# marqo-ai/marqo

Measured on AMD Instinct MI355X. Metric: embeddings/sec, higher is better.
Workload: dtype bf16; 1 GPU; open_clip ViT-B/32 image tower, uint8 224x224 resident in HBM (tower-only), batch 256/GPU; global_batch=256, parallelism=dp1 (replicated weights, sharded items, RCCL all_gather of embeddings), weights=random-init (seed 0) ViT-B-32, last_block_rows=pooled

## Files before the change

include/marqo_hip.h:

```cpp
#ifndef MARQO_HIP_H
#define MARQO_HIP_H

#include <stddef.h>
#include <stdint.h>

#ifdef __cplusplus
extern "C" {
#endif

#define MQ_OK 0
#define MQ_ERR_INVALID (-1)
#define MQ_ERR_HIP (-2)
#define MQ_ERR_WORKSPACE (-3)
#define MQ_ERR_UNSUPPORTED (-4)

#define MQ_ABI_VERSION 15

#define MQ_ACT_NONE 0
#define MQ_ACT_GELU 1
#define MQ_ACT_QUICKGELU 2
#define MQ_ACT_SILU 3
#define MQ_ACT_RELU 4

#define MQ_MASK_NONE 0
// ... 254 lines not shown
int mq_attention_stats(const void* d_qkv, void* d_out, const int32_t* d_cu_seqlens, int64_t nseq, int32_t fixed_len, int32_t max_len, int32_t W,
                       int32_t heads, int32_t mask, float* d_row_part, int64_t rows, void* stream);
int mq_attention_proj_ok(int64_t nseq, int32_t fixed_len, int32_t W, int32_t heads);
int mq_attention_proj(const void* d_qkv, const void* d_w, const float* d_bias, void* d_x, float* d_rowstats, int64_t nseq, int32_t fixed_len, int32_t W,
                      int32_t heads, float eps, const void* d_pf_a, size_t pf_a_bytes, const void* d_pf_b, size_t pf_b_bytes, void* stream);
int mq_panel_gemm_ln_ok(int64_t nseq, int32_t fixed_len, int64_t N, int64_t K);
int mq_panel_gemm_ln(const void* d_x, const void* d_W, const float* d_bias, const float* d_colsum, const float* d_rowstats, void* d_out, int64_t ldc,
                     int64_t nseq, int32_t fixed_len, int64_t N, int64_t K, int flags, void* stream);
int64_t mq_gemm_band_counters(int64_t M);
int mq_gemm_bf16_rsf(const void* d_A, int64_t lda, const void* d_W, int64_t ldw, const float* d_bias, const void* d_residual, void* d_out, int64_t ldc,
                     int64_t M, int64_t N, int64_t K, int flags, float* d_partials, float* d_stats, float eps, uint32_t* d_band_ctr,
                     const void* d_pf_a, size_t pf_a_bytes, const void* d_pf_b, size_t pf_b_bytes, void* stream);
int mq_row_stats(const void* d_x_bf16, float* d_stats, int64_t rows, int32_t W, float eps, void* stream);
int mq_gemm_bf16_ln(const void* d_A, int64_t lda, const void* d_W, int64_t ldw, const float* d_bias, const float* d_colsum, const float* d_rowstats,
                    void* d_out, int64_t ldc, int64_t M, int64_t N, int64_t K, int flags, void* stream);

int mq_layernorm(const float* d_x, const int32_t* d_row_idx, const float* d_g, const float* d_b,
                 void* d_out_bf16, float* d_out_f32, int64_t rows, int32_t W, float eps, void* stream);
int mq_layernorm_ex(const void* d_x, int x_bf16, const int32_t* d_row_idx, const float* d_g, const float* d_b,
                    void* d_out_bf16, float* d_out_f32, int64_t rows, int32_t W, float eps, void* stream);

int mq_attention(const void* d_qkv, void* d_out, const int32_t* d_cu_seqlens, int64_t nseq,
                 int32_t fixed_len, int32_t max_len, int32_t W, int32_t heads, int32_t mask,
                 void* stream);

int mq_attention_bias(const void* d_qkv, void* d_out, const int32_t* d_cu_seqlens, int64_t nseq, int32_t fixed_len,
                      int32_t max_len, int32_t W, int32_t heads, const float* d_rel_bias, int32_t rel_span, void* stream);

int mq_attention_ex(const void* d_qkv, void* d_out, const int32_t* d_cu_seqlens, int64_t nseq,
                    int32_t fixed_len, int32_t max_len, int32_t W, int32_t heads, int32_t mask,
// ... 497 lines not shown
```

marqo_amd/_lib.py:

```python
from __future__ import annotations

import ctypes as C
import os
import re
import subprocess
import sys
import sysconfig
import threading
from typing import Optional
from pathlib import Path

PKG_DIR = Path(__file__).resolve().parent
CSRC_DIR = PKG_DIR / "csrc"
LIB_DIR = PKG_DIR / "lib"
LIB_PATH = Path(os.environ["MARQO_AMD_LIB"]) if os.environ.get("MARQO_AMD_LIB") else LIB_DIR / "libmarqo_hip.so"
HEADER_PATH = PKG_DIR.parent / "include" / "marqo_hip.h"
TORCH_OPS_SRC = CSRC_DIR / "torch_ops.cpp"
TORCH_OPS_PATH = LIB_DIR / "libmarqo_torch_ops.so"
STAGE_SRC = CSRC_DIR / "py_stage.cpp"
STAGE_PATH = LIB_DIR / "_mq_stage.so"

MQ_OK = 0
NO_SCRATCH_UNITS = ("rowops", "gemm_bf16", "gemm_wd", "gemm_fp8", "gemm_small", "attention", "attention_window", "attention_gqa", "attention_gqa256", "attention_relbias", "attn_proj", "panel_gemm", "embed", "convnext", "resnet", "patch_attn", "rerank", "owl_head", "temporal", "audio", "video")
ABI_VERSION = 15
# ... 222 lines not shown
    "mq_vit_workspace_bytes": (C.c_size_t, [C.POINTER(VitCfg), C.c_int64]),
    "mq_clip_text_workspace_bytes": (C.c_size_t, [C.POINTER(ClipTextCfg), C.c_int64, C.c_int64]),
    "mq_bert_workspace_bytes": (C.c_size_t, [C.POINTER(BertCfg), C.c_int64, C.c_int64]),
    "mq_encode_image_u8": (C.c_int, [C.POINTER(VitCfg), C.POINTER(VitWeights), _P, C.c_int64, _P, C.c_int, _P, C.c_size_t, _P]),
    "mq_encode_image_f32": (C.c_int, [C.POINTER(VitCfg), C.POINTER(VitWeights), _P, C.c_int64, _P, C.c_int, _P, C.c_size_t, _P]),
    "mq_encode_clip_text": (C.c_int, [C.POINTER(ClipTextCfg), C.POINTER(ClipTextWeights), _P, _P, _P, C.c_int64, _P, _P,
                                      C.c_int, _P, C.c_size_t, _P]),
    "mq_encode_bert": (C.c_int, [C.POINTER(BertCfg), C.POINTER(BertWeights), _P, _P, _P, C.c_int64, _P, C.c_int, _P,
                                 C.c_size_t, _P]),
    "mq_gemm_bf16": (C.c_int, [_P, C.c_int64, _P, C.c_int64, _P, _P, _P, C.c_int64, C.c_int64, C.c_int64, C.c_int64,
                               C.c_int, _P]),
    "mq_gemm_small_bf16": (C.c_int, [_P, C.c_int64, _P, C.c_int64, _P, _P, _P, C.c_int64, C.c_int64, C.c_int64, C.c_int64, C.c_int, _P]),
    "mq_ln_gemm_small_bf16": (C.c_int, [_P, C.c_int64, C.c_int, _P, _P, C.c_float, _P, C.c_int64, _P, _P, C.c_int64, C.c_int64, C.c_int64,
                                        C.c_int64, C.c_int, _P, _P]),
    "mq_gemm_bf16_ln": (C.c_int, [_P, C.c_int64, _P, C.c_int64, _P, _P, _P, _P, C.c_int64, C.c_int64, C.c_int64, C.c_int64, C.c_int, _P]),
    "mq_row_stats": (C.c_int, [_P, _P, C.c_int64, C.c_int32, C.c_float, _P]),
    "mq_row_stats_finalize": (C.c_int, [_P, C.c_int32, _P, C.c_int64, C.c_int32, C.c_float, _P]),
    "mq_gemm_bf16_lnrs": (C.c_int, [_P, C.c_int64, _P, C.c_int64, _P, _P, _P, _P, _P, C.c_int64, C.c_int64, C.c_int64, C.c_int64, C.c_int, _P, _P]),
    "mq_attention_stats": (C.c_int, [_P, _P, _P, C.c_int64, C.c_int32, C.c_int32, C.c_int32, C.c_int32, C.c_int32, _P, C.c_int64, _P]),
    "mq_attention_proj_ok": (C.c_int, [C.c_int64, C.c_int32, C.c_int32, C.c_int32]),
    "mq_panel_gemm_ln_ok": (C.c_int, [C.c_int64, C.c_int32, C.c_int64, C.c_int64]),
    "mq_panel_gemm_ln": (C.c_int, [_P, _P, _P, _P, _P, _P, C.c_int64, C.c_int64, C.c_int32, C.c_int64, C.c_int64, C.c_int, _P]),
    "mq_attention_proj": (C.c_int, [_P, _P, _P, _P, _P, C.c_int64, C.c_int32, C.c_int32, C.c_int32, C.c_float, _P, C.c_size_t, _P, C.c_size_t, _P]),
    "mq_gemm_bf16_rs": (C.c_int, [_P, C.c_int64, _P, C.c_int64, _P, _P, _P, C.c_int64, C.c_int64, C.c_int64, C.c_int64, C.c_int, _P, _P]),
    "mq_check_device": (C.c_int, [C.c_int]),
    "mq_gemm_band_counters": (C.c_int64, [C.c_int64]),
    "mq_gemm_bf16_rsf": (C.c_int, [_P, C.c_int64, _P, C.c_int64, _P, _P, _P, C.c_int64, C.c_int64, C.c_int64, C.c_int64, C.c_int, _P, _P, C.c_float, _P,
                                   _P, C.c_size_t, _P, C.c_size_t, _P]),
    "mq_gemm_fp8": (C.c_int, [_P, C.c_int64, _P, C.c_int64, _P, C.c_int, _P, _P, _P, _P, C.c_int64, _P, _P, C.c_int64, C.c_int64,
                              C.c_int64, C.c_int, _P]),
# ... 387 lines not shown
```

marqo_amd/csrc/attention.hip:

```cpp
#include <type_traits>
#include "attention_core.h"
#include "knobs.h"

namespace {

#ifndef MQ_ATTN_WAVES_PER_EU
#define MQ_ATTN_WAVES_PER_EU 5
#endif
#if MQ_ATTN_WAVES_PER_EU > 0
#define MQ_ATTN_OCC __attribute__((amdgpu_waves_per_eu(HD == 64 ? MQ_ATTN_WAVES_PER_EU : 1, 8)))
#else
#define MQ_ATTN_OCC
#endif
template <int MASK, bool OUT_FP8, int HD, int HS, int NW, bool BIAS = false>
__global__ __launch_bounds__(NW * 64) MQ_ATTN_OCC void attention_kernel(
    const bf16_t* __restrict__ qkv, void* __restrict__ out_v, const int32_t* __restrict__ cu,
    int fixed_len, int W, int heads, int kpad, float scale_log2e, const float* __restrict__ out_scale, float* amax_out,
    const float* __restrict__ rel_bias = nullptr, int rel_span = 0, int band = 0, float2* __restrict__ row_part = nullptr, int64_t part_ld = 0) {
    bf16_t* out = (bf16_t*)out_v;
    extern __shared__ __attribute__((aligned(16))) char smem[];
    static_assert(HS <= HD && HS % 16 == 0 && (HD == 64 || HD == 128), "head stride: multiple of 16, at most the LDS row");
    constexpr int RB = HD * 2;
    constexpr int NC = HD / 8;
    constexpr int NCS = HS / 8;
    constexpr int NKK = (HS + 31) / 32;
    constexpr int NDT = HS / 16;
    char* sK = smem;
    char* sV = smem + (size_t)kpad * RB;

// ... 6 lines not shown
    const int ld = 3 * W;
    const bf16_t* qb = qkv + (int64_t)row0 * ld + h * HS;
    const bf16_t* kb = qb + W;
    const bf16_t* vb = qb + 2 * W;
    const int nkt = (len + 63) >> 6;
    const int kp = nkt << 6;
    const int lane = threadIdx.x & 63, wave = __builtin_amdgcn_readfirstlane(threadIdx.x >> 6);

    const int nchunks = (kp + kpad - 1) / kpad;
    auto stage = [&](int c) {
        const int base = c * kpad;
        attn_stage_piece<RB, NC, NC - 1, NW, NCS>(sK, sV, kb, vb, ld, base, kp - base < kpad ? kp - base : kpad, len, lane, wave);
    };
    if (nchunks == 1) stage(0);
    const int l15 = lane & 15, g = lane >> 4;
    const int nqb = (len + 15) >> 4;
    float amax_local = 0.f;
    auto load_q = [&](int qr, int kk) -> bf16x8 {
        const int col = 8 * g + 32 * kk;
        if (HS % 32 != 0 && col >= HS) return bf16x8{0, 0, 0, 0, 0, 0, 0, 0};
        return *(const bf16x8*)(qb + (int64_t)qr * ld + col);
    };
    bf16x8 qn[NKK];
    {
        const int q0 = wave * 16 + l15;
        const int qr = q0 < len ? q0 : len - 1;
#pragma unroll
        for (int kk = 0; kk < NKK; ++kk) qn[kk] = load_q(qr, kk);
    }
    asm volatile("s_waitcnt vmcnt(0)" ::: "memory");
    __syncthreads();

    const int vkey = 4 * g + (l15 >> 2);
    const int vcol = (l15 & 3) >> 1, vhalf = (l15 & 1) << 3;

    const int nrounds = (nqb + NW - 1) / NW;
    for (int rnd = 0; rnd < nrounds; ++rnd) {
        const int qblk = rnd * NW + wave;
        const bool active = qblk < nqb;
        if (nchunks == 1 && !active) break;
        const int q = qblk * 16 + l15;
// ... 36 lines not shown
#pragma unroll
                for (int t = 0; t < 4; ++t)
#pragma unroll
                    for (int r = 0; r < 4; ++r) {
                        const int key = kt * 64 + t * 16 + g * 4 + r;
                        sc[t][r] += rb[key < len ? key : len - 1];
                    }
            }
            attn_mask_causal<MASK>(sc, kt, nkt, g, q, qblk * 16, len);
            attn_softmax_step<NDT>(sc, m_run, l_run, o, scale_log2e);
            attn_pv_tile<RB, NDT, NC - 1>(sV, kt, cb, vkey, vcol, vhalf, sc, o);
        }
        }
        if (!active) continue;
        const float inv = attn_inv_denominator(l_run);
        if (q < len) {
            if (OUT_FP8) {
                const float qs = 1.0f / out_scale[0];
                uint8_t* orow8 = (uint8_t*)out_v + (int64_t)(row0 + q) * W + h * HS + 4 * g;
#pragma unroll
                for (int dt = 0; dt < NDT; ++dt) {
                    float v[4];
#pragma unroll
                    for (int e = 0; e < 4; ++e) {
                        v[e] = o[dt][e] * inv;
                        amax_local = fmaxf(amax_local, fabsf(v[e]));
                        v[e] = fminf(fmaxf(v[e] * qs, -448.f), 448.f);
                    }
                    int w = __builtin_amdgcn_cvt_pk_fp8_f32(v[0], v[1], 0, false);
                    w = __builtin_amdgcn_cvt_pk_fp8_f32(v[2], v[3], w, true);
                    *(int*)(orow8 + dt * 16) = w;
// ... 29 lines not shown
        }
    }
    if (OUT_FP8 && amax_out) {
        amax_local = wave_max(amax_local);
        if (lane == 0) atomicMax((int*)amax_out, __float_as_int(amax_local));
    }
}


}


static int attention_impl(const void* d_qkv, void* d_out, const int32_t* d_cu_seqlens, int64_t nseq,
                          int32_t fixed_len, int32_t max_len, int32_t W, int32_t heads, int32_t mask,
                          int32_t out_fp8, const float* d_out_scale, float* d_amax, const float* d_rel_bias, int32_t rel_span, void* stream,
                          float* d_row_part = nullptr, int64_t part_ld = 0) {
    ATTN_ARG_PTRS("mq_attention", d_qkv, d_out);
    MQ_CHECK_ARG(!d_row_part || (!out_fp8 && !d_rel_bias), "mq_attention_stats: bf16 output, no relative-position bias");
    MQ_CHECK_ARG(heads >= 1 && W % heads == 0, "mq_attention: W=%d is not a multiple of heads=%d", W, heads);
    const int hs = W / heads;
    MQ_CHECK_ARG(hs == 64 || hs == 96 || hs == 112 || hs == 128, "mq_attention: head dim must be 64, 96, 112 or 128 (W=%d heads=%d)", W, heads);
    const int hd = hs == 64 ? 64 : 128;
    ATTN_ARG_SEQS("mq_attention", fixed_len, d_cu_seqlens);
    MQ_CHECK_ARG(mask == MQ_MASK_NONE || mask == MQ_MASK_CAUSAL || mask == MQ_MASK_CAUSAL_CLS, "mq_attention: bad mask %d", mask);
    MQ_CHECK_ARG(mask != MQ_MASK_CAUSAL_CLS || !out_fp8, "mq_attention: MQ_MASK_CAUSAL_CLS runs with bf16 output only");
    if (nseq <= 0) return MQ_OK;
    const int maxl = fixed_len > 0 ? fixed_len : max_len;
    ATTN_ARG_MAXL("mq_attention", maxl);
    MQ_CHECK_ARG(!d_rel_bias || (hs == 64 && mask == MQ_MASK_NONE && !out_fp8 && rel_span >= maxl),
                 "mq_attention_bias: the relative-position bias runs with 64-wide heads, no mask, bf16 output and rel_span (%d) >= the longest "
                 "sequence (%d)", rel_span, maxl);
    ATTN_ARG_GRID("mq_attention", nseq * heads);
    const int kpad = attn_kpad(maxl, hd == 64 ? 640 : 320);
    const size_t lds = (size_t)kpad * hd * 4;
    hipStream_t s = (hipStream_t)stream;
    const bool five = mq_attention_waves == 5 && maxl > 64 && maxl <= 80 && hs == 64 && !d_rel_bias;
    const int knob_waves = mq_attention_waves;
    const int nw = five ? 5 : (knob_waves == 4 || knob_waves == 8 ? knob_waves : (maxl > 128 ? 8 : 4));
    const float scale_log2e = 1.44269504088896340736f / sqrtf((float)hs);
    MqProfScope prof(2, s);
    auto launch = [&](auto kern) -> int {
        if (lds > 64 * 1024) {
            hipError_t e = hipFuncSetAttribute((const void*)kern, hipFuncAttributeMaxDynamicSharedMemorySize, (int)lds);
            if (e != hipSuccess) { mq_set_error("mq_attention: hipFuncSetAttribute: %s", hipGetErrorString(e)); return MQ_ERR_HIP; }
        }
        hipLaunchKernelGGL(kern, dim3((unsigned)(nseq * heads)), dim3(nw * 64), lds, s, (const bf16_t*)d_qkv,
                           d_out, d_cu_seqlens, (int)fixed_len, (int)W, (int)heads, kpad, scale_log2e, d_out_scale, d_amax, d_rel_bias, (int)rel_span,
                           (mq_xcd_band && nseq * heads >= 2048) ? 1 : 0, (float2*)d_row_part, part_ld);
        return MQ_OK;
    };
    if (d_rel_bias) {
        const int rcb = nw == 8 ? launch(attention_kernel<MQ_MASK_NONE, false, 64, 64, 8, true>) : launch(attention_kernel<MQ_MASK_NONE, false, 64, 64, 4, true>);
        if (rcb != MQ_OK) return rcb;
        MQ_CHECK_LAUNCH("mq_attention_bias");
        return MQ_OK;
    }
    MQ_CHECK_ARG(!out_fp8 || d_out_scale, "mq_attention: fp8 output needs an out_scale");
    int rc;
    auto pick_nw = [&](auto hd_tag, auto hs_tag, auto nw_tag) -> int {
        constexpr int HD_ = decltype(hd_tag)::value, HS_ = decltype(hs_tag)::value, NW_ = decltype(nw_tag)::value;
        if (out_fp8) return (mask == MQ_MASK_CAUSAL) ? launch(attention_kernel<MQ_MASK_CAUSAL, true, HD_, HS_, NW_>) : launch(attention_kernel<MQ_MASK_NONE, true, HD_, HS_, NW_>);
        if (mask == MQ_MASK_CAUSAL_CLS) return launch(attention_kernel<MQ_MASK_CAUSAL_CLS, false, HD_, HS_, NW_>);
        return (mask == MQ_MASK_CAUSAL) ? launch(attention_kernel<MQ_MASK_CAUSAL, false, HD_, HS_, NW_>) : launch(attention_kernel<MQ_MASK_NONE, false, HD_, HS_, NW_>);
    };
    auto pick = [&](auto hd_tag, auto hs_tag) -> int {
        if constexpr (decltype(hd_tag)::value == 64)
            if (nw == 5) return pick_nw(hd_tag, hs_tag, std::integral_constant<int, 5>{});
        return nw == 8 ? pick_nw(hd_tag, hs_tag, std::integral_constant<int, 8>{}) : pick_nw(hd_tag, hs_tag, std::integral_constant<int, 4>{});
    };
    using std::integral_constant;
    switch (hs) {
        case 64: rc = pick(integral_constant<int, 64>{}, integral_constant<int, 64>{}); break;
        case 96: rc = pick(integral_constant<int, 128>{}, integral_constant<int, 96>{}); break;
// ... 15 lines not shown
                                 int32_t max_len, int32_t W, int32_t heads, const float* d_rel_bias, int32_t rel_span, void* stream) {
    MQ_CHECK_ARG(d_rel_bias, "mq_attention_bias: null bias table");
    return attention_impl(d_qkv, d_out, d_cu_seqlens, nseq, fixed_len, max_len, W, heads, MQ_MASK_NONE, 0, nullptr, nullptr, d_rel_bias, rel_span, stream);
}

extern "C" int mq_attention(const void* d_qkv, void* d_out, const int32_t* d_cu_seqlens, int64_t nseq, int32_t fixed_len,
                            int32_t max_len, int32_t W, int32_t heads, int32_t mask, void* stream) {
    return mq_attention_ex(d_qkv, d_out, d_cu_seqlens, nseq, fixed_len, max_len, W, heads, mask, 0, nullptr, nullptr, stream);
}

extern "C" int mq_attention_stats(const void* d_qkv, void* d_out, const int32_t* d_cu_seqlens, int64_t nseq, int32_t fixed_len, int32_t max_len, int32_t W,
                                  int32_t heads, int32_t mask, float* d_row_part, int64_t rows, void* stream) {
    MQ_CHECK_ARG(d_row_part && rows >= 1 && (fixed_len <= 0 || rows == nseq * fixed_len), "mq_attention_stats: null partials / rows does not match the sequences");
    return attention_impl(d_qkv, d_out, d_cu_seqlens, nseq, fixed_len, max_len, W, heads, mask, 0, nullptr, nullptr, nullptr, 0, stream, d_row_part, rows);
}
```

marqo_amd/csrc/gemm_bf16.hip:

```cpp
#include <map>
#include <mutex>
#include <type_traits>
#include "common.h"
#include "gemm_epilogue.h"
#include "gemm_loop.h"
#include "gemm_sched.h"

bool mq_gemm_small_ok(int64_t M, int64_t N, int64_t K, bool ln);
bool mq_gemm_small_grouped_ok(int64_t M, int64_t N, int64_t K);
int mq_gemm_small(const void* d_A, int64_t lda, const void* d_W, int64_t ldw, const float* d_bias, const void* d_residual, void* d_out,
                  int64_t ldc, int64_t M, int64_t N, int64_t K, int flags, hipStream_t s);
int mq_gemm_wd_launch(int flags, int mt, int ns, const void* A, int64_t lda, const void* W, int64_t ldw, const float* bias, const float* residual, void* out,
                      int64_t ldc, int M, int N, int K, const GemmGeom& g, int wide, const GemmLn& ln, hipStream_t s);

int mq_device_ok();

namespace {

struct GemmSk {
    float* partials;
    unsigned* flags;
    unsigned epoch;
    int tail_splits;
};
// ... 332 lines not shown
        w.partials = (float*)p;
        w.flags = (unsigned*)((char*)p + (size_t)RESIDENT_SLOTS_WIDE * SK_SLOT_BYTES);
        if (hipError_t e = hipMemsetAsync(w.flags, 0, 4096, s); e != hipSuccess) {
            mq_set_error("mq_gemm_bf16: tail workspace memset: %s", hipGetErrorString(e));
            return MQ_ERR_HIP;
        }
    }
    if (++w.epoch == 0) w.epoch = 1;
    out.partials = w.partials;
    out.flags = w.flags;
    out.epoch = w.epoch;
    return MQ_OK;
}

GemmLn ln_rows_from(GemmLn ln, int64_t r, int64_t bands) {
    if (ln.rowstats) ln.rowstats += r;
    if (ln.partials) ln.partials += r;
    if (ln.band_ctr) { ln.band_ctr += bands; ln.stats_out += r; }
    return ln;
}

template <int FLAGS, int MT, int NH = 1, int ORD = 2, int WM = 2>
int launch_gemm_mt(const void* A, int64_t lda, const void* W, int64_t ldw, const float* bias, const float* residual, void* out, int64_t ldc,
                   int M, int N, int K, hipStream_t s, const GemmLn& ln) {
    constexpr int BM = 16 * MT * WM, BN = 128 * NH;
    constexpr int LDS = 2 * (BM + BN) * BK * 2;
    constexpr int SLOTS = (NH == 1 && WM == 2) ? RESIDENT_SLOTS : RESIDENT_SLOTS_WIDE;
    static std::atomic<uint64_t> attr_done{0};
    auto kern = gemm_nt_kernel<FLAGS, MT, NH, WM, ORD>;
    if (hipError_t e = mq_ensure_dyn_lds((const void*)kern, LDS, attr_done); e != hipSuccess) {
        mq_set_error("mq_gemm_bf16: hipFuncSetAttribute: %s", hipGetErrorString(e));
// ... 150 lines not shown
        MQ_GEMM_CASE(MQ_EPI_BIAS | MQ_EPI_OUT_F32);
        MQ_GEMM_CASE(MQ_EPI_BIAS);
        MQ_GEMM_CASE(MQ_EPI_BIAS | MQ_EPI_GELU);
        MQ_GEMM_CASE(MQ_EPI_BIAS | MQ_EPI_GELU | MQ_EPI_OUT_F32);
        MQ_GEMM_CASE(MQ_EPI_BIAS | MQ_EPI_QUICKGELU);
        MQ_GEMM_CASE(MQ_EPI_BIAS | MQ_EPI_RESIDUAL | MQ_EPI_OUT_F32);
        MQ_GEMM_CASE(MQ_EPI_BIAS | MQ_EPI_RESIDUAL);
        MQ_GEMM_CASE(MQ_EPI_BIAS | MQ_EPI_GLU);
        default:
            mq_set_error("mq_gemm_bf16: unsupported epilogue flag combination 0x%x", flags);
            return MQ_ERR_INVALID;
    }
#undef MQ_GEMM_CASE
}

extern "C" int mq_gemm_bf16_ln(const void* d_A, int64_t lda, const void* d_W, int64_t ldw, const float* d_bias, const float* d_colsum,
                               const float* d_rowstats, void* d_out, int64_t ldc, int64_t M, int64_t N, int64_t K, int flags, void* stream) {
    MQ_CHECK_ARG(d_A && d_W && d_out && d_bias && d_colsum && d_rowstats, "mq_gemm_bf16_ln: null operand");
    MQ_TRY(check_shape("mq_gemm_bf16_ln", M, N, K, lda, ldw, ldc));
    MQ_CHECK_ARG(!(flags & MQ_EPI_GLU) || N % 32 == 0, "mq_gemm_bf16_ln: MQ_EPI_GLU needs N %% 32 == 0");
    hipStream_t s = (hipStream_t)stream;
    MqProfScope prof(0, s, 2.0 * (double)M * (double)N * (double)K);
    const int m = (int)M, n = (int)N, k = (int)K;
    GemmLn ln{};
    ln.colsum = d_colsum;
    ln.rowstats = (const float2*)d_rowstats;
#define MQ_GEMM_LN_CASE(F) \
    case (F): return launch_gemm<(F)>(d_A, lda, d_W, ldw, d_bias, nullptr, d_out, ldc, m, n, k, s, ln)
    switch (flags | MQ_EPI_LN_APPLY) {
        MQ_GEMM_LN_CASE(MQ_EPI_BIAS | MQ_EPI_LN_APPLY);
        MQ_GEMM_LN_CASE(MQ_EPI_BIAS | MQ_EPI_GELU | MQ_EPI_LN_APPLY);
        MQ_GEMM_LN_CASE(MQ_EPI_BIAS | MQ_EPI_QUICKGELU | MQ_EPI_LN_APPLY);
        MQ_GEMM_LN_CASE(MQ_EPI_BIAS | MQ_EPI_RELU | MQ_EPI_LN_APPLY);
        MQ_GEMM_LN_CASE(MQ_EPI_BIAS | MQ_EPI_GLU | MQ_EPI_LN_APPLY);
        default:
            mq_set_error("mq_gemm_bf16_ln: unsupported epilogue flag combination 0x%x", flags);
            return MQ_ERR_INVALID;
    }
#undef MQ_GEMM_LN_CASE
}

extern "C" int mq_gemm_bf16_rs(const void* d_A, int64_t lda, const void* d_W, int64_t ldw, const float* d_bias, const void* d_residual, void* d_out,
                               int64_t ldc, int64_t M, int64_t N, int64_t K, int flags, float* d_partials, void* stream) {
    MQ_CHECK_ARG(d_A && d_W && d_out && d_bias && d_residual && d_partials, "mq_gemm_bf16_rs: null operand");
    MQ_CHECK_ARG((flags | MQ_EPI_ROW_STATS) == (MQ_EPI_BIAS | MQ_EPI_RESIDUAL | MQ_EPI_ROW_STATS), "mq_gemm_bf16_rs: flags must be MQ_EPI_BIAS | MQ_EPI_RESIDUAL");
    MQ_TRY(check_shape("mq_gemm_bf16_rs", M, N, K, lda, ldw, ldc));
    hipStream_t s = (hipStream_t)stream;
    MqProfScope prof(0, s, 2.0 * (double)M * (double)N * (double)K);
    GemmLn ln{};
    ln.partials = (float2*)d_partials;
    ln.nslots = (int)((N + 63) / 64);
    ln.part_ld = M;
    return launch_gemm<MQ_EPI_BIAS | MQ_EPI_RESIDUAL | MQ_EPI_ROW_STATS>(d_A, lda, d_W, ldw, d_bias, (const float*)d_residual, d_out, ldc, (int)M, (int)N, (int)K, s, ln);
}
// ... 57 lines not shown
```

marqo_amd/csrc/gemm_epilogue.h:

```cpp
#pragma once
#include "common.h"

struct GemmLn {
    const float* colsum;
    const float2* rowstats;
    float2* partials;
    int nslots;
    int64_t part_ld;
    unsigned* band_ctr;
    float2* stats_out;
    float inv_w, eps;
    int band_target;
    const unsigned* pf_a;
    const unsigned* pf_b;
    unsigned pf_na, pf_nb;
};

__device__ __forceinline__ void gemm_pf_issue(const GemmLn& ln, unsigned (&pf_regs)[2]) {
    const unsigned nt = gridDim.x * blockDim.x, t = blockIdx.x * blockDim.x + threadIdx.x;
#pragma unroll
    for (int j = 0; j < 2; ++j) {
        const unsigned c = t + j * nt;
        const unsigned* src = c < ln.pf_na ? ln.pf_a + (size_t)c * 32 : (c - ln.pf_na < ln.pf_nb ? ln.pf_b + (size_t)(c - ln.pf_na) * 32 : nullptr);
        if (src) asm volatile("global_load_dword %0, %1, off" : "=v"(pf_regs[j]) : "v"(src) : "memory");
// ... 42 lines not shown
    constexpr bool LN_APPLY = (FLAGS & MQ_EPI_LN_APPLY) != 0, ROW_STATS = (FLAGS & MQ_EPI_ROW_STATS) != 0, GLU = (FLAGS & MQ_EPI_GLU) != 0;
    static_assert(!GLU || (BF16_OUT && !(FLAGS & (MQ_EPI_RESIDUAL | MQ_EPI_GELU | MQ_EPI_QUICKGELU))), "GLU: bias (+ LN apply, + row statistics of the product), bf16 out");
    static_assert(!ROW_STATS || RES_BF16 || GLU, "ROW_STATS rides on the bf16 read-modify-write residual epilogue or on the gated product");
    static_assert(!LN_APPLY || (BF16_OUT && (!(FLAGS & MQ_EPI_RESIDUAL) || RES_BF16)), "LN_APPLY: bf16 out (QKV / fc1, or the bf16 residual epilogue)");
    float row_mean = 0.f, row_rstd = 1.f;
    asm volatile("" ::: "memory");
    __builtin_amdgcn_sched_barrier(0);
    f32x4 res_v[(FLAGS & MQ_EPI_RESIDUAL) ? RG : 1][4];
    constexpr bool LN_RES = LN_APPLY && (FLAGS & MQ_EPI_RESIDUAL) != 0;
    float2 ms_g[LN_RES ? RG : 1];
    auto prefetch_residual = [&](int mt_lo) {
        if (FLAGS & MQ_EPI_RESIDUAL) {
#pragma unroll
            for (int h = 0; h < RG; ++h) {
                const int m = wave_m0 + (mt_lo + h) * 16 + l15;
                if constexpr (LN_RES) ms_g[h] = (mt_lo + h < MT && m < M) ? lnp->rowstats[m] : make_float2(0.f, 1.f);
#pragma unroll
                for (int nt = 0; nt < 4; ++nt) {
                    const int n = wave_n0 + nt * 16 + g * 4;
                    if (RES_BF16) {
                        uint2 q = make_uint2(0u, 0u);
                        if (mt_lo + h < MT && m < M && n < N) q = *(const uint2*)((const bf16_t*)residual + (int64_t)m * ldc + n);
                        res_v[h][nt] = f32x4{__uint_as_float(q.x << 16), __uint_as_float(q.x & 0xffff0000u), __uint_as_float(q.y << 16),
                                             __uint_as_float(q.y & 0xffff0000u)};
                    } else {
                        res_v[h][nt] = (mt_lo + h < MT && m < M && n < N) ? *(const f32x4*)(residual + (int64_t)m * ldc + n)
                                                                        : f32x4{0.f, 0.f, 0.f, 0.f};
                    }
                }
            }
        }
    };
    prefetch_residual(0);
    f32x4 bias_v[4], cs_v[4];
#pragma unroll
    for (int nt = 0; nt < 4; ++nt) {
        const int n = wave_n0 + nt * 16 + g * 4;
        if ((FLAGS & MQ_EPI_BIAS) && lds_bias) bias_v[nt] = *(const f32x4*)(lds_bias + nt * 16 + g * 4);
        else bias_v[nt] = ((FLAGS & MQ_EPI_BIAS) && n < N) ? *(const f32x4*)(bias + n) : f32x4{0.f, 0.f, 0.f, 0.f};
        cs_v[nt] = (LN_APPLY && n < N) ? *(const f32x4*)(lnp->colsum + n) : f32x4{0.f, 0.f, 0.f, 0.f};
    }
    float2 ms_v[(LN_APPLY && !LN_RES) ? MT : 1];
    if (LN_APPLY && !LN_RES) {
#pragma unroll
        for (int mt = 0; mt < MT; ++mt) {
            const int m = wave_m0 + mt * 16 + l15;
            ms_v[mt] = m < M ? lnp->rowstats[m] : make_float2(0.f, 1.f);
        }
    }
    if (WAIT_LOADS) __builtin_amdgcn_s_waitcnt(0x0F70);
    auto value = [&](int mt, int nt, int m, int n, bool ok) {
        f32x4 v = acc[mt][nt];
        if (LN_APPLY) {
#pragma unroll
            for (int e = 0; e < 4; ++e) v[e] = row_rstd * (v[e] - row_mean * cs_v[nt][e]);
        }
        if (FLAGS & MQ_EPI_BIAS) v += bias_v[nt];
        if (FLAGS & MQ_EPI_GELU) {
            v = gelu_erf4(v);
        }
        if (FLAGS & MQ_EPI_QUICKGELU) {
#pragma unroll
// ... 119 lines not shown
```

marqo_amd/csrc/knobs.h:

```cpp
#pragma once
#include <atomic>
#include <stdint.h>

typedef std::atomic<int> mq_knob;

struct GemmTune { mq_knob mt, cgroup, nh, fp8_big, tail, wd, rs_fin; };
extern GemmTune g_tune;
extern std::atomic<uint64_t> mq_gemm_addr_limit;

extern mq_knob mq_tower_row_select, mq_tower_ln_fold, mq_tower_subln_fold, mq_tower_attn_proj, mq_tower_panel_gemm, mq_tower_residual_bf16,
    mq_tower_pool_strided, mq_tower_assemble_stats;
extern mq_knob mq_gemm_small_max_rows, mq_gemm_small_group_rows;
extern mq_knob mq_ln_prefetch, mq_ln_rows_per_wave, mq_ln_bf16_wide;
extern mq_knob mq_xcd_band;
extern mq_knob mq_attention_waves;
```

marqo_amd/csrc/knobs.hip:

```cpp
#include <stdlib.h>
#include <string.h>
#include "common.h"
#include "knobs.h"

GemmTune g_tune;
std::atomic<uint64_t> mq_gemm_addr_limit{0xffffffffull};
mq_knob mq_tower_row_select, mq_tower_ln_fold, mq_tower_subln_fold, mq_tower_attn_proj, mq_tower_panel_gemm, mq_tower_residual_bf16,
    mq_tower_pool_strided, mq_tower_assemble_stats;
mq_knob mq_gemm_small_max_rows, mq_gemm_small_group_rows;
mq_knob mq_ln_prefetch, mq_ln_rows_per_wave, mq_ln_bf16_wide;
mq_knob mq_xcd_band;
mq_knob mq_attention_waves;

namespace {

struct Knob { const char* key; const char* env; int def; mq_knob* var; };
const Knob g_knobs[] = {
    {"gemm_mt", "MQ_GEMM_MT", 0, &g_tune.mt},
    {"gemm_cgroup", "MQ_GEMM_CGROUP", 8, &g_tune.cgroup},
    {"gemm_nh", "MQ_GEMM_NH", 0, &g_tune.nh},
    {nullptr, "MQ_GEMM_FP8_NH", 0, &g_tune.fp8_big},
    {"gemm_tail", "MQ_GEMM_TAIL", 0, &g_tune.tail},
    {"gemm_wd", "MQ_GEMM_WD", 0, &g_tune.wd},
    {"rs_finalize", "MQ_GEMM_RS_FIN", 0, &g_tune.rs_fin},
    {"row_select", "MQ_ROW_SELECT", 1, &mq_tower_row_select},
    {"ln_fold", "MQ_LN_FOLD", 2, &mq_tower_ln_fold},
    {"subln_fold", "MQ_SUBLN_FOLD", 1, &mq_tower_subln_fold},
    {"attn_proj", "MQ_ATTN_PROJ", 128, &mq_tower_attn_proj},
    {"panel_gemm", "MQ_PANEL_GEMM", 0, &mq_tower_panel_gemm},
    {"residual_bf16", "MQ_RESIDUAL_BF16", 0, &mq_tower_residual_bf16},
    {"pool_strided", "MQ_POOL_STRIDED", 1, &mq_tower_pool_strided},
    {"assemble_stats", "MQ_ASSEMBLE_STATS", 1, &mq_tower_assemble_stats},
    {"small_m", "MQ_SMALL_M", 80, &mq_gemm_small_max_rows},
    {"small_m_grouped", "MQ_SMALL_M_GROUPED", 320, &mq_gemm_small_group_rows},
    {"ln_prefetch", "MQ_LN_PREFETCH", 1, &mq_ln_prefetch},
    {"ln_rows", "MQ_LN_ROWS", 2, &mq_ln_rows_per_wave},
    {"ln_bf16_wide", "MQ_LN_BF16_WIDE", 1, &mq_ln_bf16_wide},
    {"xcd_band", "MQ_XCD_BAND", 1, &mq_xcd_band},
    {"attn_waves", nullptr, 0, &mq_attention_waves},
    {"gemm_addr_limit_mb", nullptr, 0, nullptr},
};

const bool g_knobs_from_env = [] {
    for (const Knob& k : g_knobs) {
        const char* v = k.env ? getenv(k.env) : nullptr;
        if (k.var) *k.var = v ? atoi(v) : k.def;
    }
// ... 30 lines not shown
```

marqo_amd/csrc/towers.hip:

```cpp
#include "packed_text.h"
#include "knobs.h"

int mq_cast_bf16(const float* d_x, void* d_out, int64_t n, hipStream_t s);
extern "C" int mq_rowquant_fp8(const float* d_x, void* d_out_fp8, float* d_row_scale, int64_t rows, int32_t W, void* stream);

static_assert(sizeof(mq_block_weights) == 36 * 8, "mq_block_weights layout");
static_assert(sizeof(mq_encoder_cfg) == 112, "mq_encoder_cfg layout");
static_assert(sizeof(mq_vit_cfg) == 168 && sizeof(mq_clip_text_cfg) == 128 && sizeof(mq_bert_cfg) == 136, "tower cfg layouts");
static_assert(sizeof(mq_vit_weights) == 11 * 8 && sizeof(mq_map_head) == 11 * 8 && sizeof(mq_clip_text_weights) == 7 * 8, "tower weight layouts");

static bool attn_proj_fill_ok(int64_t nseq) {
    const int64_t rounds = (nseq + 255) / 256;
    return mq_tower_attn_proj > 0 && nseq >= mq_tower_attn_proj && (rounds == 1 || nseq * 4 >= rounds * 256 * 3);
}
static bool panel_fill_ok(int64_t nseq) {
    const int64_t rounds = (nseq + 255) / 256;
    return mq_tower_panel_gemm > 0 && nseq >= mq_tower_panel_gemm && nseq * 4 >= rounds * 256 * 3;
}
extern "C" int mq_layernorm_ex(const void* d_x, int x_bf16, const int32_t* d_row_idx, const float* d_g, const float* d_b, void* d_out_bf16,
                               float* d_out_f32, int64_t rows, int32_t W, float eps, void* stream);
bool mq_gemm_small_ok(int64_t M, int64_t N, int64_t K, bool ln);
int mq_ln_gemm_small(const void* d_x, int64_t ldx, int x_bf16, const float* ln_g, const float* ln_b, float eps, const void* d_W, int64_t ldw,
                     const float* d_bias, void* d_out, int64_t ldc, int64_t M, int64_t N, int64_t K, int flags, float* d_ln_out,
                     const int32_t* d_rows, hipStream_t s);
// ... 13 lines not shown
int mq_gemm_small(const void* d_A, int64_t lda, const void* d_W, int64_t ldw, const float* d_bias, const void* d_residual, void* d_out, int64_t ldc, int64_t M,
                  int64_t N, int64_t K, int flags, hipStream_t s);
static inline int act_epi(int act) { return act == MQ_ACT_QUICKGELU ? MQ_EPI_QUICKGELU : act == MQ_ACT_RELU ? MQ_EPI_RELU : MQ_EPI_GELU; }
extern "C" int mq_gemm_bf16_ln(const void* d_A, int64_t lda, const void* d_W, int64_t ldw, const float* d_bias, const float* d_colsum,
                               const float* d_rowstats, void* d_out, int64_t ldc, int64_t M, int64_t N, int64_t K, int flags, void* stream);
extern "C" int mq_gemm_bf16_rs(const void* d_A, int64_t lda, const void* d_W, int64_t ldw, const float* d_bias, const void* d_residual, void* d_out,
                               int64_t ldc, int64_t M, int64_t N, int64_t K, int flags, float* d_partials, void* stream);
extern "C" int mq_gemm_bf16_rsf(const void* d_A, int64_t lda, const void* d_W, int64_t ldw, const float* d_bias, const void* d_residual, void* d_out,
                                int64_t ldc, int64_t M, int64_t N, int64_t K, int flags, float* d_partials, float* d_stats, float eps,
                                uint32_t* d_band_ctr, const void* d_pf_a, size_t pf_a_bytes, const void* d_pf_b, size_t pf_b_bytes, void* stream);
extern "C" int64_t mq_gemm_band_counters(int64_t M);
bool mq_gemm_rs_in_launch();
int mq_row_stats_finalize_pf(const float* d_partials, int32_t nslots, float* d_stats, int64_t rows, int32_t W, float eps, const void* pf_a, size_t bytes_a,
                             const void* pf_b, size_t bytes_b, hipStream_t s);
bool mq_row_stats_ok(int32_t W);
int mq_row_stats_pf(const void* d_x_bf16, float* d_stats, int64_t rows, int32_t W, float eps, const void* pf_a, size_t bytes_a, const void* pf_b,
                    size_t bytes_b, hipStream_t s);
bool mq_vit_assemble_stats_ok(int32_t W);
int mq_vit_assemble_stats(const float* d_patch_out, const float* cls, const float* pos, const float* g, const float* b, void* d_x, float* d_stats, int64_t n,
                          int32_t T, int32_t W, float eps, const void* pf_a, size_t bytes_a, const void* pf_b, size_t bytes_b, hipStream_t s);
static bool fold_ok(int xb, const void* wf, const float* bf, const float* sf, int64_t rows, int N, int K) {
    return mq_tower_ln_fold && xb && wf && bf && sf && mq_row_stats_ok(K) && !mq_gemm_small_ok(rows, N, K, false) && !mq_gemm_small_grouped_ok(rows, N, K);
}
static int ln_gemm(const void* d_x, int xb, const float* g, const float* b, float eps, void* h, const void* W, const float* bias, void* out,
                   int64_t rows, int N, int K, int flags, hipStream_t s, const void* next_w = nullptr, size_t next_bytes = 0,
                   const void* wf = nullptr, const float* bf = nullptr, const float* sf = nullptr, float* row_stats = nullptr,
                   bool stats_ready = false ) {
    if (mq_gemm_small_ok(rows, N, K, true)) return mq_ln_gemm_small(d_x, K, xb, g, b, eps, W, K, bias, out, N, rows, N, K, flags, nullptr, nullptr, s);
    if (row_stats && fold_ok(xb, wf, bf, sf, rows, N, K)) {
        if (!stats_ready) MQ_TRY(mq_row_stats_pf(d_x, row_stats, rows, K, eps, pf(wf), (size_t)N * K * 2, pf(next_w), next_bytes, s));
// ... 135 lines not shown
        const int rflags = xb ? (MQ_EPI_BIAS | MQ_EPI_RESIDUAL) : res_flags;
        MQ_TRY(mq_layernorm_fp8_pf(d_x, xb, b.ln1_g, b.ln1_b, h, row_scale, nullptr, rows, W, cfg->ln_eps, pf(b.qkv_w8), (size_t)3 * Wa * W, nullptr, 0, s));
        MQ_TRY(mq_gemm_fp8(h, W, b.qkv_w8, W, row_scale, 1, b.qkv_ws, b.qkv_b, nullptr, qf, 3 * Wa, nullptr, nullptr, rows, 3 * Wa, W,
                           MQ_EPI_BIAS, s));
        MQ_TRY(mq_attention_ex(qf, a, d_cu_seqlens, nseq, fixed_len, max_len, Wa, cfg->heads, cfg->mask, 1, s_attn, nullptr, s));
        MQ_TRY(mq_move_rows(a, d_sel, h, nsel, (int64_t)Wa, false, s));
        MQ_TRY(mq_move_rows(d_x, d_sel, x_sel, nsel, (int64_t)W * (xb ? 2 : 4), false, s));
        MQ_TRY(mq_gemm_fp8(h, Wa, b.out_w8, Wa, s_attn, 0, b.out_ws, b.out_b, x_sel, x_sel, W, nullptr, nullptr, nsel, W, Wa, rflags, s));
        MQ_TRY(mq_layernorm_fp8_ex(x_sel, xb, b.ln2_g, b.ln2_b, a, row_scale, nullptr, nsel, W, cfg->ln_eps, s));
        MQ_TRY(mq_gemm_fp8(a, W, b.fc1_w8, W, row_scale, 1, b.fc1_ws, b.fc1_b, nullptr, qf, F, s_mlp, nullptr, nsel, F, W, act8, s));
        MQ_TRY(mq_gemm_fp8(qf, F, b.fc2_w8, F, s_mlp, 0, b.fc2_ws, b.fc2_b, x_sel, x_sel, W, nullptr, nullptr, nsel, W, F, rflags, s));
    } else if (!cfg->post_ln) {
        const int xb = stream_bf16(cfg) ? 1 : 0;
        const int rflags = xb ? (MQ_EPI_BIAS | MQ_EPI_RESIDUAL) : res_flags;
        const int64_t xrow = (int64_t)W * (xb ? 2 : 4);
        MQ_TRY(ln_gemm(d_x, xb, b.ln1_g, b.ln1_b, cfg->ln_eps, h, b.qkv_w, b.qkv_b, qf, rows, 3 * Wa, W, MQ_EPI_BIAS, s, nullptr, 0, b.qkv_wf, b.qkv_bf, b.qkv_sf, row_stats, stats_ready));
        MQ_TRY(attn_bf16(cfg, qf, a, d_cu_seqlens, nseq, fixed_len, max_len, Wa, s));
        if (sel_stride > 0) {
            const int64_t lda = sel_stride * Wa, ldx = sel_stride * W;
            MQ_TRY(mq_gemm_bf16(a, lda, b.out_w, Wa, b.out_b, d_x, d_x, ldx, nsel, W, Wa, rflags, s));
            if (mq_gemm_small_ok(nsel, F, W, true))
                MQ_TRY(mq_ln_gemm_small(d_x, ldx, xb, b.ln2_g, b.ln2_b, cfg->ln_eps, b.fc1_w, W, b.fc1_b, qf, F, nsel, F, W, MQ_EPI_BIAS | act_flag, nullptr, nullptr, s));
            else {
                MQ_TRY(mq_layernorm_rows_pf(d_x, xb, nullptr, sel_stride, b.ln2_g, b.ln2_b, h, nullptr, nsel, W, cfg->ln_eps, pf(b.fc1_w), (size_t)F * W * 2, nullptr, 0, s));
                if (act_flag & MQ_EPI_RELU) MQ_TRY(mq_gemm_small(h, W, b.fc1_w, W, b.fc1_b, nullptr, qf, F, nsel, F, W, MQ_EPI_BIAS | act_flag, s));
                else MQ_TRY(mq_gemm_bf16(h, W, b.fc1_w, W, b.fc1_b, nullptr, qf, F, nsel, F, W, MQ_EPI_BIAS | act_flag, s));
            }
            MQ_TRY(mq_gemm_bf16(qf, F, b.fc2_w, F, b.fc2_b, d_x, d_x, ldx, nsel, W, F, rflags, s));
            return MQ_OK;
        }
        MQ_TRY(mq_move_rows(a, d_sel, h, nsel, (int64_t)Wa * 2, false, s));
        MQ_TRY(mq_move_rows(d_x, d_sel, x_sel, nsel, xrow, false, s));
// ... 332 lines not shown
                                  const int32_t* d_cu_seqlens, int64_t nseq, int32_t fixed_len, int32_t max_len,
                                  void* d_workspace, size_t workspace_bytes, void* stream) {
    return encoder_forward_impl(cfg, blocks, d_x, rows, d_cu_seqlens, nseq, fixed_len, max_len, nullptr, 0, d_workspace, workspace_bytes,
                                (hipStream_t)stream);
}

extern "C" int mq_encoder_forward_rows(const mq_encoder_cfg* cfg, const mq_block_weights* blocks, float* d_x, int64_t rows,
                                       const int32_t* d_cu_seqlens, int64_t nseq, int32_t fixed_len, int32_t max_len,
                                       const int32_t* d_out_rows, int64_t n_out_rows, void* d_workspace, size_t workspace_bytes,
                                       void* stream) {
    MQ_CHECK_ARG(d_out_rows && n_out_rows > 0, "mq_encoder_forward_rows: empty row selection");
    return encoder_forward_impl(cfg, blocks, d_x, rows, d_cu_seqlens, nseq, fixed_len, max_len, d_out_rows, n_out_rows, d_workspace,
                                workspace_bytes, (hipStream_t)stream);
}

namespace {
struct VitPlan {
    int T, np, Kp; int64_t rows;
    size_t off_x, off_rows, off_cls, off_stats0, off_enc, off_patches, off_patch_out, total;
    size_t off_map_y, off_map_z, off_map_h, off_tok, off_kv;
};
VitPlan vit_plan(const mq_vit_cfg* c, int64_t n) {
    VitPlan p;
    const int G = c->image_size / c->patch_size;
    const bool map = c->pool == MQ_VIT_POOL_MAP || c->pool == MQ_VIT_POOL_QUERY;
    p.np = G * G; p.T = p.np + (c->pool == MQ_VIT_POOL_MAP ? 0 : 1); p.Kp = ceil64(3 * c->patch_size * c->patch_size); p.rows = n * p.T;
    const int W = c->enc.width;
    Off cv;
    p.off_x = cv.take((size_t)p.rows * W * 4);
    p.off_rows = cv.take((size_t)n * 4);
// ... 291 lines not shown
```

Before: 94900 embeddings/s.

## Compute only class-token query and attention in pooled last ViT block

In the last encoder block, when only the class-token row per sequence is pooled, the QKV projection is split. K and V are computed for every row, but Q is computed only for the first row of each sequence, using a strided row-statistics GEMM variant. A Q0 specialization of the attention kernel then runs a single query block and writes only row 0. This removes about a third of the last block's QKV GEMM work and most of its attention work, at the cost of an extra GEMM launch and new code paths gated by a knob that defaults on.

```diff
diff --git a/include/marqo_hip.h b/include/marqo_hip.h
--- a/include/marqo_hip.h
+++ b/include/marqo_hip.h
@@ -292,6 +292,11 @@
 int mq_row_stats(const void* d_x_bf16, float* d_stats, int64_t rows, int32_t W, float eps, void* stream);
 int mq_gemm_bf16_ln(const void* d_A, int64_t lda, const void* d_W, int64_t ldw, const float* d_bias, const float* d_colsum, const float* d_rowstats,
                     void* d_out, int64_t ldc, int64_t M, int64_t N, int64_t K, int flags, void* stream);
+int mq_gemm_bf16_ln_rows(const void* d_A, int64_t lda, const void* d_W, int64_t ldw, const float* d_bias, const float* d_colsum, const float* d_rowstats,
+                         int64_t rowstats_stride, void* d_out, int64_t ldc, int64_t M, int64_t N, int64_t K, int flags, void* stream);
+int mq_encoder_forward_first_rows(const mq_encoder_cfg* cfg, const mq_block_weights* blocks, float* d_x, int64_t rows, int64_t nseq, int32_t fixed_len,
+                                  void* d_workspace, size_t workspace_bytes, void* stream);
+int mq_attention_first(const void* d_qkv, void* d_out, int64_t nseq, int32_t fixed_len, int32_t W, int32_t heads, void* stream);
 
 int mq_layernorm(const float* d_x, const int32_t* d_row_idx, const float* d_g, const float* d_b,
                  void* d_out_bf16, float* d_out_f32, int64_t rows, int32_t W, float eps, void* stream);
diff --git a/marqo_amd/_lib.py b/marqo_amd/_lib.py
--- a/marqo_amd/_lib.py
+++ b/marqo_amd/_lib.py
@@ -260,6 +260,9 @@
     "mq_ln_gemm_small_bf16": (C.c_int, [_P, C.c_int64, C.c_int, _P, _P, C.c_float, _P, C.c_int64, _P, _P, C.c_int64, C.c_int64, C.c_int64,
                                         C.c_int64, C.c_int, _P, _P]),
     "mq_gemm_bf16_ln": (C.c_int, [_P, C.c_int64, _P, C.c_int64, _P, _P, _P, _P, C.c_int64, C.c_int64, C.c_int64, C.c_int64, C.c_int, _P]),
+    "mq_gemm_bf16_ln_rows": (C.c_int, [_P, C.c_int64, _P, C.c_int64, _P, _P, _P, C.c_int64, _P, C.c_int64, C.c_int64, C.c_int64, C.c_int64, C.c_int, _P]),
+    "mq_encoder_forward_first_rows": (C.c_int, [C.POINTER(EncoderCfg), C.POINTER(BlockWeights), _P, C.c_int64, C.c_int64, C.c_int32, _P, C.c_size_t, _P]),
+    "mq_attention_first": (C.c_int, [_P, _P, C.c_int64, C.c_int32, C.c_int32, C.c_int32, _P]),
     "mq_row_stats": (C.c_int, [_P, _P, C.c_int64, C.c_int32, C.c_float, _P]),
     "mq_row_stats_finalize": (C.c_int, [_P, C.c_int32, _P, C.c_int64, C.c_int32, C.c_float, _P]),
     "mq_gemm_bf16_lnrs": (C.c_int, [_P, C.c_int64, _P, C.c_int64, _P, _P, _P, _P, _P, C.c_int64, C.c_int64, C.c_int64, C.c_int64, C.c_int, _P, _P]),
diff --git a/marqo_amd/csrc/attention.hip b/marqo_amd/csrc/attention.hip
--- a/marqo_amd/csrc/attention.hip
+++ b/marqo_amd/csrc/attention.hip
@@ -12,7 +12,7 @@
 #else
 #define MQ_ATTN_OCC
 #endif
-template <int MASK, bool OUT_FP8, int HD, int HS, int NW, bool BIAS = false>
+template <int MASK, bool OUT_FP8, int HD, int HS, int NW, bool BIAS = false, bool Q0 = false>
 __global__ __launch_bounds__(NW * 64) MQ_ATTN_OCC void attention_kernel(
     const bf16_t* __restrict__ qkv, void* __restrict__ out_v, const int32_t* __restrict__ cu,
     int fixed_len, int W, int heads, int kpad, float scale_log2e, const float* __restrict__ out_scale, float* amax_out,
@@ -49,7 +49,7 @@
     };
     if (nchunks == 1) stage(0);
     const int l15 = lane & 15, g = lane >> 4;
-    const int nqb = (len + 15) >> 4;
+    const int nqb = Q0 ? 1 : (len + 15) >> 4;
     float amax_local = 0.f;
     auto load_q = [&](int qr, int kk) -> bf16x8 {
         const int col = 8 * g + 32 * kk;
@@ -59,7 +59,7 @@
     bf16x8 qn[NKK];
     {
         const int q0 = wave * 16 + l15;
-        const int qr = q0 < len ? q0 : len - 1;
+        const int qr = Q0 ? 0 : q0 < len ? q0 : len - 1;
 #pragma unroll
         for (int kk = 0; kk < NKK; ++kk) qn[kk] = load_q(qr, kk);
     }
@@ -126,7 +126,7 @@
         }
         if (!active) continue;
         const float inv = attn_inv_denominator(l_run);
-        if (q < len) {
+        if (Q0 ? q == 0 : q < len) {
             if (OUT_FP8) {
                 const float qs = 1.0f / out_scale[0];
                 uint8_t* orow8 = (uint8_t*)out_v + (int64_t)(row0 + q) * W + h * HS + 4 * g;
@@ -186,7 +186,7 @@
 static int attention_impl(const void* d_qkv, void* d_out, const int32_t* d_cu_seqlens, int64_t nseq,
                           int32_t fixed_len, int32_t max_len, int32_t W, int32_t heads, int32_t mask,
                           int32_t out_fp8, const float* d_out_scale, float* d_amax, const float* d_rel_bias, int32_t rel_span, void* stream,
-                          float* d_row_part = nullptr, int64_t part_ld = 0) {
+                          float* d_row_part = nullptr, int64_t part_ld = 0, bool first_only = false) {
     ATTN_ARG_PTRS("mq_attention", d_qkv, d_out);
     MQ_CHECK_ARG(!d_row_part || (!out_fp8 && !d_rel_bias), "mq_attention_stats: bf16 output, no relative-position bias");
     MQ_CHECK_ARG(heads >= 1 && W % heads == 0, "mq_attention: W=%d is not a multiple of heads=%d", W, heads);
@@ -208,7 +208,7 @@
     hipStream_t s = (hipStream_t)stream;
     const bool five = mq_attention_waves == 5 && maxl > 64 && maxl <= 80 && hs == 64 && !d_rel_bias;
     const int knob_waves = mq_attention_waves;
-    const int nw = five ? 5 : (knob_waves == 4 || knob_waves == 8 ? knob_waves : (maxl > 128 ? 8 : 4));
+    const int nw = first_only ? 4 : five ? 5 : (knob_waves == 4 || knob_waves == 8 ? knob_waves : (maxl > 128 ? 8 : 4));
     const float scale_log2e = 1.44269504088896340736f / sqrtf((float)hs);
     MqProfScope prof(2, s);
     auto launch = [&](auto kern) -> int {
@@ -229,6 +229,12 @@
     }
     MQ_CHECK_ARG(!out_fp8 || d_out_scale, "mq_attention: fp8 output needs an out_scale");
     int rc;
+    if (first_only) {
+        rc = launch(attention_kernel<MQ_MASK_NONE, false, 64, 64, 4, false, true>);
+        if (rc != MQ_OK) return rc;
+        MQ_CHECK_LAUNCH("mq_attention_first");
+        return MQ_OK;
+    }
     auto pick_nw = [&](auto hd_tag, auto hs_tag, auto nw_tag) -> int {
         constexpr int HD_ = decltype(hd_tag)::value, HS_ = decltype(hs_tag)::value, NW_ = decltype(nw_tag)::value;
         if (out_fp8) return (mask == MQ_MASK_CAUSAL) ? launch(attention_kernel<MQ_MASK_CAUSAL, true, HD_, HS_, NW_>) : launch(attention_kernel<MQ_MASK_NONE, true, HD_, HS_, NW_>);
@@ -274,3 +280,11 @@
     MQ_CHECK_ARG(d_row_part && rows >= 1 && (fixed_len <= 0 || rows == nseq * fixed_len), "mq_attention_stats: null partials / rows does not match the sequences");
     return attention_impl(d_qkv, d_out, d_cu_seqlens, nseq, fixed_len, max_len, W, heads, mask, 0, nullptr, nullptr, nullptr, 0, stream, d_row_part, rows);
 }
+
+bool mq_attention_first_ok(int32_t fixed_len, int32_t W, int32_t heads, int32_t mask) {
+    return fixed_len >= 1 && fixed_len <= 64 && heads >= 1 && W == heads * 64 && mask == MQ_MASK_NONE;
+}
+extern "C" int mq_attention_first(const void* d_qkv, void* d_out, int64_t nseq, int32_t fixed_len, int32_t W, int32_t heads, void* stream) {
+    MQ_CHECK_ARG(mq_attention_first_ok(fixed_len, W, heads, MQ_MASK_NONE), "mq_attention_first: fixed_len %d must lie in [1, 64] and W = %d be %d heads of 64", fixed_len, W, heads);
+    return attention_impl(d_qkv, d_out, nullptr, nseq, fixed_len, fixed_len, W, heads, MQ_MASK_NONE, 0, nullptr, nullptr, nullptr, 0, stream, nullptr, 0, true);
+}
diff --git a/marqo_amd/csrc/gemm_bf16.hip b/marqo_amd/csrc/gemm_bf16.hip
--- a/marqo_amd/csrc/gemm_bf16.hip
+++ b/marqo_amd/csrc/gemm_bf16.hip
@@ -370,7 +370,7 @@
 }
 
 GemmLn ln_rows_from(GemmLn ln, int64_t r, int64_t bands) {
-    if (ln.rowstats) ln.rowstats += r;
+    if (ln.rowstats) ln.rowstats += r * ln.rs_stride;
     if (ln.partials) ln.partials += r;
     if (ln.band_ctr) { ln.band_ctr += bands; ln.stats_out += r; }
     return ln;
@@ -551,9 +551,11 @@
 #undef MQ_GEMM_CASE
 }
 
-extern "C" int mq_gemm_bf16_ln(const void* d_A, int64_t lda, const void* d_W, int64_t ldw, const float* d_bias, const float* d_colsum,
-                               const float* d_rowstats, void* d_out, int64_t ldc, int64_t M, int64_t N, int64_t K, int flags, void* stream) {
+extern "C" int mq_gemm_bf16_ln_rows(const void* d_A, int64_t lda, const void* d_W, int64_t ldw, const float* d_bias, const float* d_colsum,
+                                    const float* d_rowstats, int64_t rowstats_stride, void* d_out, int64_t ldc, int64_t M, int64_t N, int64_t K, int flags,
+                                    void* stream) {
     MQ_CHECK_ARG(d_A && d_W && d_out && d_bias && d_colsum && d_rowstats, "mq_gemm_bf16_ln: null operand");
+    MQ_CHECK_ARG(rowstats_stride >= 1 && rowstats_stride < (1 << 30), "mq_gemm_bf16_ln: bad row-statistics stride %ld", (long)rowstats_stride);
     MQ_TRY(check_shape("mq_gemm_bf16_ln", M, N, K, lda, ldw, ldc));
     MQ_CHECK_ARG(!(flags & MQ_EPI_GLU) || N % 32 == 0, "mq_gemm_bf16_ln: MQ_EPI_GLU needs N %% 32 == 0");
     hipStream_t s = (hipStream_t)stream;
@@ -562,6 +564,7 @@
     GemmLn ln{};
     ln.colsum = d_colsum;
     ln.rowstats = (const float2*)d_rowstats;
+    ln.rs_stride = (int)rowstats_stride;
 #define MQ_GEMM_LN_CASE(F) \
     case (F): return launch_gemm<(F)>(d_A, lda, d_W, ldw, d_bias, nullptr, d_out, ldc, m, n, k, s, ln)
     switch (flags | MQ_EPI_LN_APPLY) {
@@ -575,6 +578,10 @@
             return MQ_ERR_INVALID;
     }
 #undef MQ_GEMM_LN_CASE
+}
+extern "C" int mq_gemm_bf16_ln(const void* d_A, int64_t lda, const void* d_W, int64_t ldw, const float* d_bias, const float* d_colsum,
+                               const float* d_rowstats, void* d_out, int64_t ldc, int64_t M, int64_t N, int64_t K, int flags, void* stream) {
+    return mq_gemm_bf16_ln_rows(d_A, lda, d_W, ldw, d_bias, d_colsum, d_rowstats, 1, d_out, ldc, M, N, K, flags, stream);
 }
 
 extern "C" int mq_gemm_bf16_rs(const void* d_A, int64_t lda, const void* d_W, int64_t ldw, const float* d_bias, const void* d_residual, void* d_out,
diff --git a/marqo_amd/csrc/gemm_epilogue.h b/marqo_amd/csrc/gemm_epilogue.h
--- a/marqo_amd/csrc/gemm_epilogue.h
+++ b/marqo_amd/csrc/gemm_epilogue.h
@@ -4,6 +4,7 @@
 struct GemmLn {
     const float* colsum;
     const float2* rowstats;
+    int rs_stride = 1;
     float2* partials;
     int nslots;
     int64_t part_ld;
@@ -80,7 +81,7 @@
 #pragma unroll
             for (int h = 0; h < RG; ++h) {
                 const int m = wave_m0 + (mt_lo + h) * 16 + l15;
-                if constexpr (LN_RES) ms_g[h] = (mt_lo + h < MT && m < M) ? lnp->rowstats[m] : make_float2(0.f, 1.f);
+                if constexpr (LN_RES) ms_g[h] = (mt_lo + h < MT && m < M) ? lnp->rowstats[(int64_t)m * lnp->rs_stride] : make_float2(0.f, 1.f);
 #pragma unroll
                 for (int nt = 0; nt < 4; ++nt) {
                     const int n = wave_n0 + nt * 16 + g * 4;
@@ -111,7 +112,7 @@
 #pragma unroll
         for (int mt = 0; mt < MT; ++mt) {
             const int m = wave_m0 + mt * 16 + l15;
-            ms_v[mt] = m < M ? lnp->rowstats[m] : make_float2(0.f, 1.f);
+            ms_v[mt] = m < M ? lnp->rowstats[(int64_t)m * lnp->rs_stride] : make_float2(0.f, 1.f);
         }
     }
     if (WAIT_LOADS) __builtin_amdgcn_s_waitcnt(0x0F70);
diff --git a/marqo_amd/csrc/knobs.h b/marqo_amd/csrc/knobs.h
--- a/marqo_amd/csrc/knobs.h
+++ b/marqo_amd/csrc/knobs.h
@@ -9,7 +9,7 @@
 extern std::atomic<uint64_t> mq_gemm_addr_limit;
 
 extern mq_knob mq_tower_row_select, mq_tower_ln_fold, mq_tower_subln_fold, mq_tower_attn_proj, mq_tower_panel_gemm, mq_tower_residual_bf16,
-    mq_tower_pool_strided, mq_tower_assemble_stats;
+    mq_tower_pool_strided, mq_tower_assemble_stats, mq_tower_pool_first_query;
 extern mq_knob mq_gemm_small_max_rows, mq_gemm_small_group_rows;
 extern mq_knob mq_ln_prefetch, mq_ln_rows_per_wave, mq_ln_bf16_wide;
 extern mq_knob mq_xcd_band;
diff --git a/marqo_amd/csrc/knobs.hip b/marqo_amd/csrc/knobs.hip
--- a/marqo_amd/csrc/knobs.hip
+++ b/marqo_amd/csrc/knobs.hip
@@ -6,7 +6,7 @@
 GemmTune g_tune;
 std::atomic<uint64_t> mq_gemm_addr_limit{0xffffffffull};
 mq_knob mq_tower_row_select, mq_tower_ln_fold, mq_tower_subln_fold, mq_tower_attn_proj, mq_tower_panel_gemm, mq_tower_residual_bf16,
-    mq_tower_pool_strided, mq_tower_assemble_stats;
+    mq_tower_pool_strided, mq_tower_assemble_stats, mq_tower_pool_first_query;
 mq_knob mq_gemm_small_max_rows, mq_gemm_small_group_rows;
 mq_knob mq_ln_prefetch, mq_ln_rows_per_wave, mq_ln_bf16_wide;
 mq_knob mq_xcd_band;
@@ -31,6 +31,7 @@
     {"residual_bf16", "MQ_RESIDUAL_BF16", 0, &mq_tower_residual_bf16},
     {"pool_strided", "MQ_POOL_STRIDED", 1, &mq_tower_pool_strided},
     {"assemble_stats", "MQ_ASSEMBLE_STATS", 1, &mq_tower_assemble_stats},
+    {"pool_first_query", "MQ_POOL_FIRST_QUERY", 1, &mq_tower_pool_first_query},
     {"small_m", "MQ_SMALL_M", 80, &mq_gemm_small_max_rows},
     {"small_m_grouped", "MQ_SMALL_M_GROUPED", 320, &mq_gemm_small_group_rows},
     {"ln_prefetch", "MQ_LN_PREFETCH", 1, &mq_ln_prefetch},
diff --git a/marqo_amd/csrc/towers.hip b/marqo_amd/csrc/towers.hip
--- a/marqo_amd/csrc/towers.hip
+++ b/marqo_amd/csrc/towers.hip
@@ -51,6 +51,7 @@
 int mq_row_stats_finalize_pf(const float* d_partials, int32_t nslots, float* d_stats, int64_t rows, int32_t W, float eps, const void* pf_a, size_t bytes_a,
                              const void* pf_b, size_t bytes_b, hipStream_t s);
 bool mq_row_stats_ok(int32_t W);
+bool mq_attention_first_ok(int32_t fixed_len, int32_t W, int32_t heads, int32_t mask);
 int mq_row_stats_pf(const void* d_x_bf16, float* d_stats, int64_t rows, int32_t W, float eps, const void* pf_a, size_t bytes_a, const void* pf_b,
                     size_t bytes_b, hipStream_t s);
 bool mq_vit_assemble_stats_ok(int32_t W);
@@ -216,8 +217,17 @@
         const int xb = stream_bf16(cfg) ? 1 : 0;
         const int rflags = xb ? (MQ_EPI_BIAS | MQ_EPI_RESIDUAL) : res_flags;
         const int64_t xrow = (int64_t)W * (xb ? 2 : 4);
-        MQ_TRY(ln_gemm(d_x, xb, b.ln1_g, b.ln1_b, cfg->ln_eps, h, b.qkv_w, b.qkv_b, qf, rows, 3 * Wa, W, MQ_EPI_BIAS, s, nullptr, 0, b.qkv_wf, b.qkv_bf, b.qkv_sf, row_stats, stats_ready));
-        MQ_TRY(attn_bf16(cfg, qf, a, d_cu_seqlens, nseq, fixed_len, max_len, Wa, s));
+        if (mq_tower_pool_first_query && sel_stride > 0 && sel_stride == fixed_len && nsel == nseq && rows == nseq * fixed_len && !d_cu_seqlens && !cfg->d_rel_bias &&
+            mq_attention_first_ok(fixed_len, Wa, cfg->heads, cfg->mask) && row_stats && !mq_gemm_small_ok(rows, 3 * Wa, W, true) && fold_ok(xb, b.qkv_wf, b.qkv_bf, b.qkv_sf, rows, 3 * Wa, W)) {
+            if (!stats_ready) MQ_TRY(mq_row_stats_pf(d_x, row_stats, rows, W, cfg->ln_eps, pf(b.qkv_wf), (size_t)3 * Wa * W * 2, nullptr, 0, s));
+            const bf16_t* wf = (const bf16_t*)b.qkv_wf;
+            MQ_TRY(mq_gemm_bf16_ln(d_x, W, wf + (size_t)Wa * W, W, b.qkv_bf + Wa, b.qkv_sf + Wa, row_stats, (bf16_t*)qf + Wa, 3 * Wa, rows, 2 * Wa, W, MQ_EPI_BIAS, s));
+            MQ_TRY(mq_gemm_bf16_ln_rows(d_x, sel_stride * W, wf, W, b.qkv_bf, b.qkv_sf, row_stats, sel_stride, qf, sel_stride * 3 * Wa, nsel, Wa, W, MQ_EPI_BIAS, s));
+            MQ_TRY(mq_attention_first(qf, a, nseq, fixed_len, Wa, cfg->heads, s));
+        } else {
+            MQ_TRY(ln_gemm(d_x, xb, b.ln1_g, b.ln1_b, cfg->ln_eps, h, b.qkv_w, b.qkv_b, qf, rows, 3 * Wa, W, MQ_EPI_BIAS, s, nullptr, 0, b.qkv_wf, b.qkv_bf, b.qkv_sf, row_stats, stats_ready));
+            MQ_TRY(attn_bf16(cfg, qf, a, d_cu_seqlens, nseq, fixed_len, max_len, Wa, s));
+        }
         if (sel_stride > 0) {
             const int64_t lda = sel_stride * Wa, ldx = sel_stride * W;
             MQ_TRY(mq_gemm_bf16(a, lda, b.out_w, Wa, b.out_b, d_x, d_x, ldx, nsel, W, Wa, rflags, s));
@@ -580,6 +590,14 @@
                                 workspace_bytes, (hipStream_t)stream);
 }
 
+extern "C" int mq_encoder_forward_first_rows(const mq_encoder_cfg* cfg, const mq_block_weights* blocks, float* d_x, int64_t rows, int64_t nseq, int32_t fixed_len,
+                                             void* d_workspace, size_t workspace_bytes, void* stream) {
+    MQ_CHECK_ARG(cfg && nseq > 0 && fixed_len > 0 && rows == nseq * fixed_len, "mq_encoder_forward_first_rows: rows must be nseq * fixed_len");
+    MQ_TRY(check_encoder_cfg(cfg));
+    MQ_CHECK_ARG(sel_strided_ok(cfg, nseq, fixed_len), "mq_encoder_forward_first_rows: this encoder / batch does not take its pooled rows in place (mq_encoder_forward_rows)");
+    return encoder_forward_impl(cfg, blocks, d_x, rows, nullptr, nseq, fixed_len, fixed_len, nullptr, nseq, d_workspace, workspace_bytes, (hipStream_t)stream, fixed_len);
+}
+
 namespace {
 struct VitPlan {
     int T, np, Kp; int64_t rows;
```

Result: no change. 94850 embeddings/s (-0.1%).
